# uthree/tinyvc

Measured on AMD Instinct MI355X. Metric: audio-samples/sec (16 kHz) end-to-end VC, higher is better.
Workload: dtype f32 (fp32 in / out / accumulate; channel contractions as two-term fp16 splits on v_mfma_f32_32x32x16_f16: 22-bit significands, three part-products per fp32 product)

## Files before the change

tinyvc_amd/csrc/decoder.hip:

```cpp
#include "conv3s.h"
#include "conv_s2.h"
#include "film_s2.h"
#include "gemm_s2.h"
#include "small_kernels.h"
#include "tvc_common.h"

namespace tvc {


__device__ __forceinline__ float div24k(float x) {
    const float r = 1.0f / 24000.0f;
    const float q0 = __fmul_rn(x, r);
    return fmaf(fmaf(-q0, 24000.0f, x), r, q0);
}

__device__ __forceinline__ double wave_incl_scan(double v, int lane) {
#pragma unroll
    for (int o = 1; o < 64; o <<= 1) {
        double u = __shfl_up(v, o);
        if (lane >= o) v += u;
    }
    return v;
}

static __global__ __launch_bounds__(256) void harm_frame_sum_kernel(const float* __restrict__ f0, double* __restrict__ csum,
                                                                    int T, float scale, RagDev rg) {
    const int b = blockIdx.y, lane = threadIdx.x & 63;
    const int t = 4 * blockIdx.x + (threadIdx.x >> 6);
    const int rs = T;
    long fbase = (long)b * T, cbase = (long)b * kHarm * T;
    if (rg.tb) {
        T = rg.tb[b];
        fbase = cbase = rg.pre[b];
        scale = __fdiv_rn((float)T, (float)(T * kHop));
    }
    if (t >= T) return;
    const float* f = f0 + fbase;
    double acc[kHarm];
#pragma unroll
    for (int m = 0; m < kHarm; ++m) acc[m] = 0.0;
    if (lane < kHop / 8) {
#pragma unroll
        for (int k = 0; k < 8; ++k) {
            Lerp c = lerp_coord(t * kHop + 8 * lane + k, scale, T);
            float fs = lerp_eval(c, f[c.i0], f[c.i1]);
#pragma unroll
            for (int m = 0; m < kHarm; ++m) acc[m] += (double)div24k(__fmul_rn(fs, (float)(m + 1)));
        }
    }
#pragma unroll
    for (int m = 0; m < kHarm; ++m) {
        double v = acc[m];
#pragma unroll
        for (int o = 32; o > 0; o >>= 1) v += __shfl_xor(v, o);
        if (lane == m) csum[cbase + (long)m * rs + t] = v;
    }
}

static __global__ __launch_bounds__(64) void harm_frame_scan_kernel(double* __restrict__ csum, int T, RagDev rg) {
    double* p = csum + ((long)blockIdx.y * kHarm + blockIdx.x) * T;
    if (rg.tb) {
        p = csum + (long)blockIdx.x * T + rg.pre[blockIdx.y];
        T = rg.tb[blockIdx.y];
    }
    const int lane = threadIdx.x;
    double carry = 0.0;
    for (int base = 0; base < T; base += 64) {
        int i = base + lane;
        double v = i < T ? p[i] : 0.0;
        double inc = wave_incl_scan(v, lane);
        if (i < T) p[i] = carry + (inc - v);
        carry += __shfl(inc, 63);
    }
}

static __global__ __launch_bounds__(256) void harm_synth_kernel(const float* __restrict__ f0, const float* __restrict__ amps,
                                                                const double* __restrict__ coff, float* __restrict__ source,
                                                                int T, float scale_size, float scale_amp, RagDev rg) {
    const int b = blockIdx.y, lane = threadIdx.x & 63;
    const int t = 4 * blockIdx.x + (threadIdx.x >> 6);
    const int rs = T;
    const long Ls = (long)T * kHop;
    long fbase = (long)b * T, abase = (long)b * kHarm * T, sbase = (long)b * 16 * Ls;
    if (rg.tb) {
        T = rg.tb[b];
        fbase = abase = rg.pre[b];
        sbase = (long)rg.pre[b] * kHop;
        scale_size = __fdiv_rn((float)T, (float)(T * kHop));
    }
    if (t >= T) return;
    const bool act = lane < kHop / 8;
    const float* f = f0 + fbase;
    const int p0 = t * kHop + 8 * (act ? lane : 0);
    float fs[8], uv[8];
    Lerp ca[8];
#pragma unroll
    for (int e = 0; e < 8; ++e) {
        const Lerp c = lerp_coord(p0 + e, scale_size, T);
        const float a0 = f[c.i0], a1 = f[c.i1];
        fs[e] = lerp_eval(c, a0, a1);
        uv[e] = lerp_eval(c, a0 > 20.f ? 1.f : 0.f, a1 > 20.f ? 1.f : 0.f);
        ca[e] = lerp_coord(p0 + e, scale_amp, T);
    }
    for (int m = 0; m < kHarm; ++m) {
        double d[8], sum = 0.0;
#pragma unroll
        for (int e = 0; e < 8; ++e) {
            d[e] = act ? (double)div24k(__fmul_rn(fs[e], (float)(m + 1))) : 0.0;
            sum += d[e];
        }
        const double inc = wave_incl_scan(sum, lane);
        double run = coff[abase + (long)m * rs + t] + (inc - sum);
        if (act) {
            const float* am = amps + abase + (long)m * rs;
            float o[8];
#pragma unroll
            for (int e = 0; e < 8; ++e) {
                run += d[e];
                const float I = (float)run;
                const float frac = I - floorf(I);
                const float theta = __fmul_rn(6.2831854820251465f, frac);
                const float hsin = __fmul_rn(sincos_small(theta).x, uv[e]);
                const float amp = lerp_eval(ca[e], am[ca[e].i0], am[ca[e].i1]);
                o[e] = __fmul_rn(hsin, amp);
            }
            float4* dst = reinterpret_cast<float4*>(source + sbase + (long)m * Ls + p0);
            dst[0] = make_float4(o[0], o[1], o[2], o[3]);
            dst[1] = make_float4(o[4], o[5], o[6], o[7]);
        }
    }
}

static __global__ __launch_bounds__(256) void noise_ola_kernel(const float* __restrict__ frames, float* __restrict__ source, int B, int T, float* __restrict__ smax, RagDev rg) {
    __shared__ float red[4];
    const long Ls = (long)T * kHop;
    const long b = blockIdx.y;
    long fbase = b * T, sbase = (b * 16 + 15) * Ls;
    if (rg.tb) {
        T = rg.tb[b];
        fbase = rg.pre[b];
        sbase = 15 * Ls + (long)rg.pre[b] * kHop;
    }
    const long L = (long)T * kHop;
    float mx = 0.f;
    for (long i = blockIdx.x * (long)blockDim.x + threadIdx.x; i < L; i += (long)gridDim.x * blockDim.x) {
        int p = (int)i;
        int q = p + kNfft / 2;
        int f_hi = q / kHop;
        if (f_hi > T) f_hi = T;
        int f_lo = (q - (kNfft - 1) + kHop - 1) / kHop;
        if (q - (kNfft - 1) <= 0) f_lo = 0;
        float s = 0.f;
        for (int f = f_lo > 1 ? f_lo : 1; f <= f_hi; ++f)
            s = __fadd_rn(s, frames[(fbase + (f - 1)) * kNfft + (q - f * kHop)]);
        const float v = s / (float)(f_hi - f_lo + 1);
        source[sbase + p] = v;
        mx = fmaxf(mx, fabsf(v));
    }
    amax_flush_wg(smax + b, mx, red);
}

static int run_source_net(tvc_ctx* ctx, hipStream_t s, Ws& ws, const float* content, const float* f0,
                          const float* energy, float* amps, float* kern, int B, int T, const float* cmax, float* xmax_zeroed, hipEvent_t amps_ready = nullptr) {
    const int ncols = B * T;
    float* ef = ws.get<float>((size_t)B * T);
    float* x = ws.get<float>((size_t)B * kSrcCh * T);
    const int NB = ctx->rag ? ctx->rag->B : B;
    float* xmax = xmax_zeroed ? xmax_zeroed : ws.get<float>((size_t)NB);
    if (!ws.dry) {
        hipLaunchKernelGGL(window_max_kernel, dim3(grid_for((long)ncols * 64)), dim3(256), 0, s, energy, ef, (long)B, T, kHop);
        EpiSumCond ep{x, ctx->src_content_in.bias, ef, f0, ctx->src_e_w, ctx->src_e_b, ctx->src_f_w, ctx->src_f_b, kSrcCh, T, ncols};
        int rc = 0;
        if (!gemm_s2_try(&rc, ctx, s, ctx->src_content_in, content, B, kSslDim, T, 0, ep, cmax)) rc = gemm_s_launch<2, 4, 2>(ctx, s, ctx->src_content_in, content, B, kSslDim, T, 0, ep, cmax);
        TVC_CHECK(rc);
    }
    if (!ws.dry && !xmax_zeroed) TVC_HIP(ctx, hipMemsetAsync(xmax, 0, (size_t)NB * sizeof(float), s));
    for (int i = 0; i < 3; ++i) TVC_CHECK(run_convnext(ctx, s, ws, ctx->src_mid[i], x, B, T, i == 2 ? xmax : nullptr));
    if (ws.dry) return 0;
    EpiBias<ACT_ELU1, false> ea{amps, ctx->src_to_amps.bias, nullptr, kHarm, T, ncols, (long)kHarm * T, 0};
    TVC_CHECK((gemm_s_launch<1, 4, 2>(ctx, s, ctx->src_to_amps, x, B, kSrcCh, T, 0, ea, xmax)));
    if (amps_ready) TVC_HIP(ctx, hipEventRecord(amps_ready, s));
    EpiBias<ACT_ELU1, false> ek{kern, ctx->src_to_kernel.bias, nullptr, kBins, T, ncols, (long)kBins * T, 0};
    TVC_CHECK((gemm_s_launch<2, 4, 2>(ctx, s, ctx->src_to_kernel, x, B, kSrcCh, T, 0, ek, xmax)));
    return launch_check(ctx, "source_net");
}

static int run_harm_sums(tvc_ctx* ctx, hipStream_t s, const float* f0, double* csum, int B, int T) {
    const long L = (long)T * kHop;
    const int NB = ctx->rag ? ctx->rag->B : B;
    const int Tg = ctx->rag ? ctx->rag->Tlong : T;
    RagDev rg;
    TVC_CHECK(rag_view(ctx, s, 1, 0, &rg, nullptr));
    const float scale_size = (float)T / (float)L;
    hipLaunchKernelGGL(harm_frame_sum_kernel, dim3((Tg + 3) / 4, NB), dim3(256), 0, s, f0, csum, T, scale_size, rg);
    hipLaunchKernelGGL(harm_frame_scan_kernel, dim3(kHarm, NB), dim3(64), 0, s, csum, T, rg);
    return launch_check(ctx, "harm_sums");
}

int run_dsp(tvc_ctx* ctx, hipStream_t s, Ws& ws, const float* f0, const float* amps, const float* kern, const float* angle, uint64_t seed, float* source, int B, int T,
            float* smax, double* csum, const DspFork* fk) {
    const long L = (long)T * kHop;
    if (!csum) csum = ws.get<double>((size_t)B * kHarm * T);
    float* frames = ws.get<float>((size_t)B * T * kNfft);
    const int NB = ctx->rag ? ctx->rag->B : B;
    const int Tg = ctx->rag ? ctx->rag->Tlong : T;
    float* smax_own = smax ? nullptr : ws.get<float>((size_t)NB);
    if (ws.dry) return 0;
    if (!smax) {
        smax = smax_own;
        TVC_HIP(ctx, hipMemsetAsync(smax, 0, (size_t)NB * sizeof(float), s));
    }
    RagDev rg;
    TVC_CHECK(rag_view(ctx, s, 1, 0, &rg, nullptr));
    const float scale_size = (float)T / (float)L;
    const float scale_amp = (float)(1.0 / (double)kHop);
    hipStream_t sh = s;
    if (fk) {
        sh = fk->side;
        TVC_HIP(ctx, hipStreamWaitEvent(sh, fk->amps_ready, 0));
    } else {
        TVC_CHECK(run_harm_sums(ctx, s, f0, csum, B, T));
    }
    hipLaunchKernelGGL(harm_synth_kernel, dim3((Tg + 3) / 4, NB), dim3(256), 0, sh, f0, amps, csum, source, T, scale_size, scale_amp, rg);
    TVC_CHECK(run_amax_rows(ctx, sh, amps, B, kHarm, T, smax));
    TVC_CHECK(run_noise_ifft(ctx, s, kern, angle, seed, frames, B, T, ctx->rag && angle));
    hipLaunchKernelGGL(noise_ola_kernel, dim3(grid_for((long)Tg * kHop / 4, 256, NB >= 32 ? 16 : 512 / NB), NB), dim3(256), 0, s, frames, source, B, T, smax, rg);
    return launch_check(ctx, "dsp");
}

static int plain_conv(tvc_ctx* ctx, hipStream_t s, const PackedW& w, const float* x, int B, int Cin, int len, int dil, float* y, const BfpSlots& bfp, int lin = 0,
                      float lscale = 0.f) {
    int rc = 0;
    if ((lin > 0 ? conv_s2_try<true>(&rc, ctx, s, w, x, B, Cin, len, dil, y, bfp, lin, lscale) : conv_s2_try<false>(&rc, ctx, s, w, x, B, Cin, len, dil, y, bfp)))
        return rc;
    if (lin > 0)
        return conv3s_launch<true, C3EpiBias<false>, false, true>(ctx, s, w, x, B, Cin, len, dil, C3EpiBias<false>{y, w.bias, nullptr, w.M, len}, bfp, nullptr, nullptr,
                                                                   nullptr, 0, lin, lscale);
    return conv3s_launch<true>(ctx, s, w, x, B, Cin, len, dil, C3EpiBias<false>{y, w.bias, nullptr, w.M, len}, bfp);
}

static int film_conv(tvc_ctx* ctx, hipStream_t s, const PackedW& w, const PackedW& fw, const FilmU& fu, const float* h, const float* cond, int B, int C, int len, int dil,
                     float* out, const float* bsc, const float* bsh, const float* res, int res_lin, float res_scale, const BfpSlots& bfp) {
    int rc = 0;
    if (rag_min_len(ctx, len) >= FS2::BN && film_s2_try(&rc, ctx, s, fu, h, cond, B, C, len, dil, out, res, res_lin, res_scale, bfp)) return rc;
    return conv3s_launch<true, C3EpiFilmFused, true>(ctx, s, w, h, B, C, len, dil, C3EpiFilmFused{out, w.bias, bsc, bsh, res, C, len, res_lin, res_scale}, bfp, &fw, &fw,
                                                     cond, C);
}

static int half_first(tvc_ctx* ctx, hipStream_t s, const PackedW& ca, const FilmU& fu, const float* x, int lin, float lscale, int da, int db, float* h, int B, int C, int len,
                      const float* res, int res_lin, const float* ma_in, float* mh, const float* mcond, bool* pre) {
    *pre = false;
    const bool can = rag_min_len(ctx, len) >= FS2::BN && fu.img && fu.C == C && fu.hb_w > 0.f && C % 96 == 0 && C <= 384 && ma_in && mcond && res && db >= 1 && db <= FS2::MAXD &&
                     (long)C * len * 4 < (1L << 32) && (res_lin <= 0 || (long)C * res_lin * 4 < (1L << 32));
    if (can) {
        int rc = 0;
        const BfpSlots in{ma_in, nullptr, nullptr};
        const bool ok = lin > 0 ? conv_s2_try<true, true>(&rc, ctx, s, ca, x, B, C, len, da, h, in, lin, lscale, fu.hb_w, fu.hb_b)
                                : conv_s2_try<false, true>(&rc, ctx, s, ca, x, B, C, len, da, h, in, 0, 0.f, fu.hb_w, fu.hb_b);
        if (ok) {
            *pre = rc == 0;
            return rc;
        }
    }
    return plain_conv(ctx, s, ca, x, B, C, len, da, h, BfpSlots{ma_in, nullptr, mh}, lin, lscale);
}

static int half_film(tvc_ctx* ctx, hipStream_t s, const PackedW& cb, const PackedW& fw, const FilmU& fu, int db, const float* h, const float* cond, int B, int C, int len,
                     float* out, const float* bsc, const float* bsh, const float* res, int res_lin, float res_scale, const float* ma_in, const float* mh, const float* mcond,
                     float* mout, bool pre) {
    if (pre) {
        int rc = 0;
        if (!film_s2_try(&rc, ctx, s, fu, h, cond, B, C, len, db, out, res, res_lin, res_scale, BfpSlots{ma_in, mcond, mout}, true, fu.hb_w, fu.hb_b))
            return fail(ctx, TVC_ERR_STATE, "filter_net: the FiLM conv refused the pre-split operand its producer wrote");
        return rc;
    }
    return film_conv(ctx, s, cb, fw, fu, h, cond, B, C, len, db, out, bsc, bsh, res, res_lin, res_scale, BfpSlots{mh, mcond, mout});
}

static int conv_film_half(tvc_ctx* ctx, hipStream_t s, const PackedW& ca, const PackedW& cb, const PackedW& fw, const FilmU& fu, const float* x, int lin, float lscale,
                          int da, int db, float* h, const float* cond, int B, int C, int len, float* out, const float* bsc, const float* bsh, const float* res,
                          int res_lin, float res_scale, const float* ma_in, float* mh, const float* mcond, float* mout) {
    bool pre = false;
    TVC_CHECK(half_first(ctx, s, ca, fu, x, lin, lscale, da, db, h, B, C, len, res, res_lin, ma_in, mh, mcond, &pre));
    return half_film(ctx, s, cb, fw, fu, db, h, cond, B, C, len, out, bsc, bsh, res, res_lin, res_scale, ma_in, mh, mcond, mout, pre);
}

constexpr int kHalfDil[2][2] = {{1, 3}, {9, 27}};

static __global__ void g8_to_planar_kernel(const float* __restrict__ x, float* __restrict__ y, long B, long l, int C) {
    const long n = B * C * l;
    for (long i = blockIdx.x * (long)blockDim.x + threadIdx.x; i < n; i += (long)gridDim.x * blockDim.x) {
        const long t = i % l, bc = i / l, c = bc % C, b = bc / C;
        y[i] = x[((b * (C / 8) + c / 8) * l + t) * 8 + (c & 7)];
    }
}

static int filter_input_gemm(tvc_ctx* ctx, hipStream_t s, const float* content, const float* f0, float* x, int B, int T, const float* cmax) {
    EpiSumCond ep{x, ctx->flt_content_in.bias, nullptr, f0, nullptr, nullptr, ctx->flt_f_w, ctx->flt_f_b, 384, T, B * T};
    int rc = 0;
    if (!gemm_s2_try(&rc, ctx, s, ctx->flt_content_in, content, B, kSslDim, T, 0, ep, cmax)) rc = gemm_s_launch<2, 4, 2>(ctx, s, ctx->flt_content_in, content, B, kSslDim, T, 0, ep, cmax);
    return rc;
}

int run_filter(tvc_ctx* ctx, hipStream_t s, Ws& ws, const float* content, const float* f0,
               const float* energy, const float* source, float* wave, int B, int T, const FilterTaps* taps, const float* cmax, const float* smax, float* zeroed_slots, bool x_slot_set,
               const FilterFront* front) {
    const long L = (long)T * kHop;
    static const int ch[5] = {384, 192, 96, 48, 24};
    const long len_dn[5] = {L, L / 5, L / 20, L / 80, L / 240};
    float* skip[5];
    for (int i = 0; i < 5; ++i) skip[i] = ws.get<float>((size_t)B * ch[4 - i] * len_dn[i]);
    float* x = front ? front->x0 : ws.get<float>((size_t)B * ch[0] * T);
    const UpW& u0 = ctx->ups[0];
    const int lo0 = T * u0.factor;
    float* h0 = front ? front->h0 : ws.get<float>((size_t)B * u0.cin * lo0);
    SideFork* fk = front && front->fk && front->fk->forked() ? front->fk : nullptr;
    bool pre0 = false;
    float* xi_pre[5] = {nullptr, nullptr, nullptr, nullptr, nullptr};
    for (int i = 1; i <= 4; ++i) xi_pre[i] = ws.get<float>((size_t)B * ctx->downs[i - 1].cin * len_dn[i]);
    for (int i = 1; i < 4; ++i)
        if (len_dn[i] % ctx->downs[i].factor != 0 || (ctx->downs[i].factor == 4 && len_dn[i] % 4 != 0))
            return fail(ctx, TVC_ERR_ARG, "filter_net: level lengths must divide by the next Downsample factor");

    enum { S_CONTENT = 0, S_SRC, S_X, S_SKIP0, S_DH1 = S_SKIP0 + 5, S_DH2 = S_DH1 + 4, S_UHA = S_DH2 + 4, S_UX1 = S_UHA + 5, S_UHB = S_UX1 + 5, S_UXU = S_UHB + 5,
           S_LEV = S_UXU + 5, S_COUNT = S_LEV + 5 };
    const int NB = ctx->rag ? ctx->rag->B : B;
    static_assert(S_COUNT == kFilterSlots && S_X == kFilterSlotX, "tvc_common.h kFilterSlots / kFilterSlotX");
    float* slots = zeroed_slots ? zeroed_slots : ws.get<float>((size_t)S_COUNT * NB);
    auto slot = [&](int i) { return slots + (size_t)i * NB; };
    auto up0_first = [&](hipStream_t st) {
        return half_first(ctx, st, u0.c1, u0.fu1, x, T, (float)(1.0 / (double)u0.factor), kHalfDil[0][0], kHalfDil[0][1], h0, B, u0.cin, lo0, x, T, slot(S_X), slot(S_UHA),
                          slot(S_SKIP0 + 4), &pre0);
    };

    if (!ws.dry) {
        ProfScope ps(ctx, s, ws, "filter.in+down0");
        if (!zeroed_slots) TVC_HIP(ctx, hipMemsetAsync(slots, 0, (size_t)S_COUNT * NB * sizeof(float), s));
        if (!cmax) {
            TVC_CHECK(run_amax_rows(ctx, s, content, B, kSslDim, T, slot(S_CONTENT)));
            cmax = slot(S_CONTENT);
        }
        if (!smax) {
            TVC_CHECK(run_amax_rows(ctx, s, source, B, 16, L, slot(S_SRC)));
            TVC_CHECK(run_amax_rows(ctx, s, energy, B, 1, L, slot(S_SRC)));
            smax = slot(S_SRC);
        }
        if (fk && !(zeroed_slots && x_slot_set)) return fail(ctx, TVC_ERR_STATE, "filter_net: a forked front needs its slots prepared in front of the fork");
        if (!fk) TVC_CHECK(filter_input_gemm(ctx, s, content, f0, x, B, T, cmax));
        if (!(zeroed_slots && x_slot_set)) TVC_CHECK(run_slot_affine(ctx, s, slot(S_X), cmax, 1, ctx->flt_in_bw, ctx->flt_in_bb, NB));
        if (fk) {
            {
                ProfScope ps(ctx, fk->side, ws, "filter_net.input@side");
                TVC_CHECK(up0_first(fk->side));
            }
            TVC_CHECK(fk->end());
        }
        TVC_CHECK(run_down0_split(ctx, s, ctx->flt_down0s, source, energy, skip[0], taps ? taps->skips[0] : nullptr, xi_pre[1], B, (int)L, smax, slot(S_SKIP0)));
    }
    for (int i = 1; i <= 4; ++i) {
        const DownW& d = ctx->downs[i - 1];
        const int len = (int)len_dn[i];
        size_t mk = ws.mark();
        float* xi = xi_pre[i];
        float* h1 = d.cin == 24 ? nullptr : ws.get<float>((size_t)B * d.cin * len);
        float* h2 = d.cin == 24 ? nullptr : ws.get<float>((size_t)B * d.cin * len);
        if (!ws.dry) {
            static const char* names[4] = {"filter.down1", "filter.down2", "filter.down3", "filter.down4"};
            ProfScope ps(ctx, s, ws, names[i - 1]);
            float* y2 = i < 4 ? xi_pre[i + 1] : nullptr;
            const int f2 = i < 4 ? ctx->downs[i].factor : 0;
            const float* mxi = slot(S_SKIP0 + i - 1);
            float *mh1 = slot(S_DH1 + i - 1), *mh2 = slot(S_DH2 + i - 1), *mout = slot(S_SKIP0 + i);
            if (d.cin == 24) {
                TVC_CHECK(run_down24_fused(ctx, s, d, xi, skip[i], y2, B, len, mxi, mout));
            } else {
                if (d.cin == 48) {
                    TVC_CHECK(run_conv48_pair(ctx, s, d.c1, d.c2, xi, 0, 0.f, nullptr, nullptr, nullptr, nullptr, h2, B, len, 1, 2, mxi, nullptr, mh2));
                } else {
                    TVC_CHECK(plain_conv(ctx, s, d.c1, xi, B, d.cin, len, 1, h1, BfpSlots{mxi, nullptr, mh1}));
                    TVC_CHECK(plain_conv(ctx, s, d.c2, h1, B, d.cin, len, 2, h2, BfpSlots{mh1, nullptr, mh2}));
                }
                TVC_CHECK((conv3s_launch<true, C3EpiBiasResConv>(ctx, s, d.c3, h2, B, d.cin, len, 4,
                                                                 C3EpiBiasResConv{{skip[i], d.c3res_bias, nullptr, d.cout, len, y2, f2}},
                                                                 BfpSlots{mh2, mxi, mout}, &d.res, nullptr, xi, d.cin)));
            }
        }
        ws.release(mk);
    }
    float* xlev[5];
    {
        long l = T;
        for (int i = 0; i < 5; ++i) {
            l *= ctx->ups[i].factor;
            xlev[i] = ws.get<float>((size_t)B * ctx->ups[i].cout * l);
        }
    }
    long len = T;
    const float* mx_in = slot(S_X);
    for (int i = 0; i < 5; ++i) {
        const UpW& u = ctx->ups[i];
        const int lin = (int)len;
        len *= u.factor;
        const int lo = (int)len, C = u.cin, nc = B * lo;
        const float* cond = skip[4 - i];
        const float* mcond = slot(S_SKIP0 + 4 - i);
        size_t mk = ws.mark();
        float* xu = ws.get<float>((size_t)B * C * lo);
        float* h = i == 0 ? h0 : ws.get<float>((size_t)B * C * lo);
        float* x1 = ws.get<float>((size_t)B * C * lo);
        if (!ws.dry && C == 24) {
            ProfScope ps(ctx, s, ws, "filter.up4+out");
            TVC_CHECK(run_up24_split(ctx, s, u, x, cond, ctx->down0_bw, ctx->down0_bb, x1, wave, B, lo, mx_in, smax, slot(S_UX1 + i)));
        } else if (!ws.dry) {
            static const char* names[4] = {"filter.up0", "filter.up1", "filter.up2", "filter.up3"};
            ProfScope ps(ctx, s, ws, names[i]);
            const float lscale = (float)(1.0 / (double)u.factor);
            for (int half = 0; half < 2; ++half) {
                const PackedW& ca = half ? u.c3 : u.c1;
                const PackedW& cb = half ? u.c4 : u.c2;
                const PackedW& fw = half ? u.film2 : u.film1;
                const float* bsc = fw.bias;
                const float* bsh = fw.bias + C;
                const int da = kHalfDil[half][0], db = kHalfDil[half][1];
                float* xout = half ? xu : x1;
                const float* ma_in = half ? slot(S_UX1 + i) : mx_in;
                float* mh = slot((half ? S_UHB : S_UHA) + i);
                float* mout = slot((half ? S_UXU : S_UX1) + i);
                if (C == 48) {
                    if (half == 0) {
                        TVC_CHECK(run_conv48_pair(ctx, s, ca, cb, x, lin, lscale, &fw, bsc, bsh, cond, xout, B, lo, da, db, ma_in, mcond, mout));
                    } else {
                        TVC_CHECK(run_conv48s(ctx, s, ca, x1, nullptr, nullptr, nullptr, nullptr, nullptr, h, B, lo, da, ma_in, nullptr, mh));
                        TVC_CHECK(run_conv48s(ctx, s, cb, h, &fw, bsc, bsh, cond, x1, nullptr, B, lo, db, mh, mcond, slot(S_LEV + i), &u.c5, xlev[i]));
                    }
                } else if (half == 0 && i == 0) {
                    if (fk) TVC_CHECK(fk->join());
                    else TVC_CHECK(up0_first(s));
                    TVC_CHECK(half_film(ctx, s, cb, fw, u.fu1, db, h, cond, B, C, lo, xout, bsc, bsh, x, lin, lscale, ma_in, mh, mcond, mout, pre0));
                } else if (half == 0) {
                    TVC_CHECK(conv_film_half(ctx, s, ca, cb, fw, u.fu1, x, lin, lscale, da, db, h, cond, B, C, lo, xout, bsc, bsh, x, lin, lscale, ma_in, mh, mcond, mout));
                } else {
                    TVC_CHECK(conv_film_half(ctx, s, ca, cb, fw, u.fu2, x1, 0, 0.f, da, db, h, cond, B, C, lo, xout, bsc, bsh, x1, 0, 0.f, ma_in, mh, mcond, mout));
                }
            }
            if (C != 48) {
                EpiBias<ACT_NONE, false> ep{xlev[i], u.c5.bias, nullptr, u.cout, lo, nc, (long)u.cout * lo, 0, slot(S_LEV + i), slot(S_UXU + i), u.c5_bw, u.c5_bb, NB};
                if (u.cout == 48) {
                    EpiBiasG8 eg{xlev[i], u.c5.bias, u.cout, lo, nc, slot(S_LEV + i), slot(S_UXU + i), u.c5_bw, u.c5_bb, NB};
                    TVC_CHECK((gemm_s_launch<2, 4, 2>(ctx, s, u.c5, xu, B, C, lo, 0, eg, slot(S_UXU + i))));
                } else if (u.c5.MT6 % 3 == 0) TVC_CHECK((gemm_s_launch<3, 4, 1>(ctx, s, u.c5, xu, B, C, lo, 0, ep, slot(S_UXU + i))));
                else TVC_CHECK((gemm_s_launch<2, 4, 2>(ctx, s, u.c5, xu, B, C, lo, 0, ep, slot(S_UXU + i))));
            }
        }
        ws.release(mk);
        x = xlev[i];
        mx_in = slot(S_LEV + i);
    }
    if (!ws.dry && taps) {
        for (int i = 1; i < 5; ++i)
            if (taps->skips[i] && i == 1)
                hipLaunchKernelGGL(g8_to_planar_kernel, dim3(grid_for((long)B * 48 * len_dn[1])), dim3(256), 0, s, skip[1], taps->skips[1], (long)B, len_dn[1], 48);
            else if (taps->skips[i])
                TVC_HIP(ctx, hipMemcpyAsync(taps->skips[i], skip[i], (size_t)B * ch[4 - i] * len_dn[i] * sizeof(float), hipMemcpyDeviceToDevice, s));
        long l = T;
        for (int i = 0; i < 4; ++i) {
            l *= ctx->ups[i].factor;
            if (taps->ups[i] && ctx->ups[i].cout <= 48)
                hipLaunchKernelGGL(g8_to_planar_kernel, dim3(grid_for((long)B * ctx->ups[i].cout * l)), dim3(256), 0, s, xlev[i], taps->ups[i], (long)B, l, ctx->ups[i].cout);
            else if (taps->ups[i])
                TVC_HIP(ctx, hipMemcpyAsync(taps->ups[i], xlev[i], (size_t)B * ctx->ups[i].cout * l * sizeof(float), hipMemcpyDeviceToDevice, s));
        }
    }
    return ws.dry ? 0 : launch_check(ctx, "filter_net");
}

int run_decoder(tvc_ctx* ctx, hipStream_t s, Ws& ws, const float* content, const float* f0,
                const float* energy, const float* angle, uint64_t seed, float* wave, float* amps_out,
                float* kernel_out, float* source_out, int B, int T, const float* content_bound, const float* energy_bound,
                int content_bound_stride) {
    const long L = (long)T * kHop;
    float* amps = amps_out ? amps_out : ws.get<float>((size_t)B * kHarm * T);
    float* kern = kernel_out ? kernel_out : ws.get<float>((size_t)B * kBins * T);
    float* source = source_out ? source_out : ws.get<float>((size_t)B * 16 * L);
    const int NB = ctx->rag ? ctx->rag->B : B;
    float* cmax = ws.get<float>((size_t)(3 + kFilterSlots) * NB);
    float* smax = cmax + NB;
    float* xmax = smax + NB;
    float* fslots = xmax + NB;
    float* x0 = ws.get<float>((size_t)B * 384 * T);
    float* h0 = ws.get<float>((size_t)B * ctx->ups[0].cin * T * ctx->ups[0].factor);
    double* csum = ws.get<double>((size_t)B * kHarm * T);
    if (!ws.dry) {
        TVC_CHECK(run_slot_prep(ctx, s, cmax, (3 + kFilterSlots) * NB, content_bound ? cmax : nullptr, content_bound, content_bound_stride, 1.f, 0.f, energy_bound ? smax : nullptr,
                                energy_bound, 1, 1.f, 0.f, content_bound ? fslots + (size_t)kFilterSlotX * NB : nullptr, ctx->flt_in_bw, ctx->flt_in_bb,
                                NB));
        if (!content_bound) TVC_CHECK(run_amax_rows(ctx, s, content, B, kSslDim, T, cmax));
        if (!energy_bound) TVC_CHECK(run_amax_rows(ctx, s, energy, B, 1, L, smax));
        if (!content_bound && wave) TVC_CHECK(run_slot_affine(ctx, s, fslots + (size_t)kFilterSlotX * NB, cmax, 1, ctx->flt_in_bw, ctx->flt_in_bb, NB));
        if (wave && ctx->rag) {
            RagDev rd;
            TVC_CHECK(rag_tiles(ctx, s, B, (long)T * ctx->ups[0].factor, CS2::BN, &rd, nullptr, "filter_net front"));
        }
    }
    SideFork fk(ctx, s);
    if (wave) TVC_CHECK(fk.fork(ws, ctx->ev_fork2, ctx->ev_join2));
    const FilterFront front{&fk, x0, h0};
    if (fk.forked()) {
        TVC_CHECK(run_harm_sums(ctx, fk.side, f0, csum, B, T));
        ProfScope ps(ctx, fk.side, ws, "filter_net.input@side");
        TVC_CHECK(filter_input_gemm(ctx, fk.side, content, f0, x0, B, T, cmax));
    }
    size_t mk = ws.mark();
    {
        ProfScope ps(ctx, s, ws, "source_net");
        TVC_CHECK(run_source_net(ctx, s, ws, content, f0, energy, amps, kern, B, T, cmax, xmax, fk.forked() ? ctx->ev_amps : nullptr));
    }
    ws.release(mk);
    if (!wave && !source_out) return 0;
    {
        ProfScope ps(ctx, s, ws, "dsp");
        const DspFork df{fk.side, ctx->ev_amps};
        TVC_CHECK(run_dsp(ctx, s, ws, f0, amps, kern, angle, seed, source, B, T, smax, csum, fk.forked() ? &df : nullptr));
        TVC_CHECK(fk.join_so_far(ctx->ev_src));
    }
    ws.release(mk);
    if (!wave) return 0;
    ProfScope ps(ctx, s, ws, "filter_net");
    TVC_CHECK(run_filter(ctx, s, ws, content, f0, energy, source, wave, B, T, nullptr, cmax, smax, fslots, true, &front));
    ws.release(mk);
    return 0;
}

}
```

tinyvc_amd/csrc/encoder.hip:

```cpp
#include "conv3s.h"
#include "gemm_s2.h"
#include "cnx_s3.h"
#include "small_kernels.h"
#include "tvc_common.h"

namespace tvc {

constexpr int ENC_MTB = 4, ENC_NWV = 4, ENC_BPC = 2;

template <bool DW, int CPT>
static __global__ __launch_bounds__(1024) void dwconv_ln_kernel(const float* x, float* y,
                                                               const float* __restrict__ dw_w, const float* __restrict__ dw_b,
                                                               const float* __restrict__ g, const float* __restrict__ bta,
                                                               int C, int T, int dil, RagDev rg) {
    constexpr int NW = 16;
    const int rs = T;
    long ubase = (long)blockIdx.y * C * T;
    if (rg.tb) {
        T = rg.tb[blockIdx.y];
        ubase = rg.pre[blockIdx.y];
        if ((int)blockIdx.x * 64 >= T) return;
    }
    __shared__ float red[NW][64];
    constexpr bool STAGE = CPT >= 16;
    __shared__ __attribute__((aligned(16))) float Wl[STAGE ? 16 * CPT * 8 : 8];
    __shared__ float Gl[2][STAGE ? 16 * CPT : 1];
    if (STAGE) {
        for (int i = threadIdx.x; i < C; i += 1024) {
            if (DW) {
#pragma unroll
                for (int j = 0; j < 7; ++j) Wl[i * 8 + j] = dw_w[i * 7 + j];
                Wl[i * 8 + 7] = dw_b[i];
            }
            Gl[0][i] = g[i];
            Gl[1][i] = bta[i];
        }
        __syncthreads();
    }
    const int lane = threadIdx.x & 63, wave = threadIdx.x >> 6;
    const int t = blockIdx.x * 64 + lane;
    const bool ok = t < T;
    const int tc = ok ? t : T - 1;
    const float* xb = x + ubase;
    float* yb = y + ubase;

    int tt[7];
#pragma unroll
    for (int j = 0; j < 7; ++j) {
        int q = tc + (j - 3) * dil;
        tt[j] = q < 0 ? 0 : (q >= T ? T - 1 : q);
    }
    float v[CPT];
    float sum = 0.f;
#pragma unroll
    for (int i = 0; i < CPT; ++i) {
        const int c = wave + i * NW;
        if (DW) {
            const float* xr = xb + (long)c * rs;
            float wj[7], a;
            if (STAGE) {
                const float4 w0 = *reinterpret_cast<const float4*>(Wl + c * 8), w1 = *reinterpret_cast<const float4*>(Wl + c * 8 + 4);
                wj[0] = w0.x; wj[1] = w0.y; wj[2] = w0.z; wj[3] = w0.w; wj[4] = w1.x; wj[5] = w1.y; wj[6] = w1.z;
                a = w1.w;
            } else {
#pragma unroll
                for (int j = 0; j < 7; ++j) wj[j] = dw_w[c * 7 + j];
                a = dw_b[c];
            }
#pragma unroll
            for (int j = 0; j < 7; ++j) a = fmaf(wj[j], xr[tt[j]], a);
            v[i] = a;
        } else {
            v[i] = xb[(long)c * rs + tc];
        }
        sum += v[i];
    }
    red[wave][lane] = sum;
    __syncthreads();
    float tot = 0.f;
#pragma unroll
    for (int w = 0; w < NW; ++w) tot += red[w][lane];
    const float mean = tot / (float)C;
    __syncthreads();
    float sq = 0.f;
#pragma unroll
    for (int i = 0; i < CPT; ++i) {
        const float d = v[i] - mean;
        sq = fmaf(d, d, sq);
    }
    red[wave][lane] = sq;
    __syncthreads();
    float tot2 = 0.f;
#pragma unroll
    for (int w = 0; w < NW; ++w) tot2 += red[w][lane];
    const float var = tot2 / (float)C;
    const float rstd = 1.f / sqrtf(var + 1e-5f);
    if (!ok) return;
#pragma unroll
    for (int i = 0; i < CPT; ++i) {
        const int c = wave + i * NW;
        yb[(long)c * rs + t] = fmaf((v[i] - mean) * rstd, STAGE ? Gl[0][c] : g[c], STAGE ? Gl[1][c] : bta[c]);
    }
}
template <bool DW>
static int dwconv_ln_launch(tvc_ctx* ctx, hipStream_t s, const float* x, float* y, const float* dw_w, const float* dw_b, const float* g,
                            const float* bta, int B, int C, int T, int dil) {
    RagDev rg;
    TVC_CHECK(rag_view(ctx, s, 1, 0, &rg, nullptr));
    const dim3 grid(((ctx->rag ? ctx->rag->Tlong : T) + 63) / 64, ctx->rag ? ctx->rag->B : B), blk(1024);
    if (C == 384) hipLaunchKernelGGL((dwconv_ln_kernel<DW, 24>), grid, blk, 0, s, x, y, dw_w, dw_b, g, bta, C, T, dil, rg);
    else if (C == 128) hipLaunchKernelGGL((dwconv_ln_kernel<DW, 8>), grid, blk, 0, s, x, y, dw_w, dw_b, g, bta, C, T, dil, rg);
    else return fail(ctx, TVC_ERR_ARG, "dwconv_ln: unsupported channel count %d", C);
    return 0;
}

static __global__ void grn_norm_kernel(const float* __restrict__ h, float* __restrict__ gx, long rows, int T, RagDev rg, int C2) {
    const int lane = threadIdx.x & 63;
    long wave = (blockIdx.x * (long)blockDim.x + threadIdx.x) >> 6;
    long nwaves = ((long)gridDim.x * blockDim.x) >> 6;
    for (long r = wave; r < rows; r += nwaves) {
        const float* p = h + r * T;
        int n = T;
        if (rg.tb) {
            const int b = (int)(r / C2), c = (int)(r - (long)b * C2);
            p = h + (long)c * T + rg.pre[b];
            n = rg.tb[b];
        }
        float s = 0.f;
        for (int t = lane; t < n; t += 64) s = fmaf(p[t], p[t], s);
#pragma unroll
        for (int o = 32; o > 0; o >>= 1) s += __shfl_xor(s, o);
        if (lane == 0) gx[r] = sqrtf(s);
    }
}

static __global__ __launch_bounds__(256) void grn_finalize_kernel(const float* __restrict__ gx, const float* __restrict__ gamma,
                                                                  float* __restrict__ nx, int C2, float* __restrict__ hmax) {
    __shared__ float red[4];
    __shared__ float redm[4];
    const int b = blockIdx.x;
    const float* g = gx + (long)b * C2;
    float s = 0.f;
    for (int c = threadIdx.x; c < C2; c += 256) s += g[c];
#pragma unroll
    for (int o = 32; o > 0; o >>= 1) s += __shfl_xor(s, o);
    if ((threadIdx.x & 63) == 0) red[threadIdx.x >> 6] = s;
    __syncthreads();
    const float mean = (red[0] + red[1] + red[2] + red[3]) / (float)C2;
    const float den = mean + 1e-6f;
    float mx = 0.f;
    for (int c = threadIdx.x; c < C2; c += 256) {
        const float f = fmaf(gamma[c], g[c] / den, 1.f);
        nx[(long)b * C2 + c] = f;
        mx = fmaxf(mx, g[c] * fabsf(f));
    }
#pragma unroll
    for (int o = 32; o > 0; o >>= 1) mx = fmaxf(mx, __shfl_xor(mx, o));
    if ((threadIdx.x & 63) == 0) redm[threadIdx.x >> 6] = mx;
    __syncthreads();
    if (threadIdx.x == 0) hmax[b] = fmaxf(fmaxf(redm[0], redm[1]), fmaxf(redm[2], redm[3]));
}

int run_layernorm(tvc_ctx* ctx, hipStream_t s, float* x, const float* g, const float* b, int B, int C, int T) {
    TVC_CHECK(dwconv_ln_launch<false>(ctx, s, x, x, nullptr, nullptr, g, b, B, C, T, 1));
    return launch_check(ctx, "layernorm");
}

static __global__ void grn_tiles_kernel(float* __restrict__ gp, int gp_tiles, int K, int T, RagDev rg) {
    const int b = blockIdx.y, c = blockIdx.x * blockDim.x + threadIdx.x;
    if (c >= K) return;
    const int Tb = rg.tb ? rg.tb[b] : T, n = (Tb + 63) / 64;
    float* g = gp + (long)b * gp_tiles * K + c;
    float s = g[0];
    for (int t = 1; t < n; ++t) s += g[(long)t * K];
    g[0] = s;
}

template <int C>
static bool cnx_try(int* rc, tvc_ctx* ctx, hipStream_t s, const ConvNeXtW& w, float* x, float* h, float* gx, int B, int T, float* amax_out) {
    if (w.C != C || !(w.ln_bound < 32768.f) || w.c2.MT6 != 2 * C / 32 || w.c3.MT6 != C / 32 || w.c2.S6 < C / 16 || w.c3.S6 < 2 * C / 16) return false;
    const int NB = ctx->rag ? ctx->rag->B : B, Tl = ctx->rag ? ctx->rag->Tlong : T, rs = T;
    if ((long)rs * 8 * 4 >= (1L << 31)) return false;
    constexpr int KP = C == 384 ? 2 : 1;
    if ((*rc = lds_optin<cnx1_kernel<C, 1>>(ctx, Cnx1<C, 1>::LDS_BYTES, "cnx")) ||
        (*rc = lds_optin<cnx1_kernel<C, 2>>(ctx, Cnx1<C, 2>::LDS_BYTES, "cnx")) ||
        (*rc = lds_optin<cnx2_kernel<C, KP>>(ctx, Cnx2<C, KP>::LDS_BYTES, "cnx")))
        return true;
    CnxArgs a{};
    a.x = x;
    a.h = h;
    a.T = T;
    a.rs = rs;
    if ((*rc = rag_view(ctx, s, 1, 0, &a.rg, nullptr)) != 0) return true;
    auto split = [&](int MT, int tiles) {
        int d = 1;
        for (int c = 1; c <= MT; ++c)
            if (MT % c == 0 && (long)tiles * c <= ctx->ncu) d = c;
        return d;
    };
    {
        a.A6 = reinterpret_cast<const uint4*>(w.c2.A6);
        a.wsc = w.c2.wscale;
        a.bias = w.c2.bias;
        a.MT = w.c2.MT6;
        a.dw_w = w.dw_w;
        a.dw_b = w.dw_b;
        a.ln_g = w.ln_g;
        a.ln_b = w.ln_b;
        a.dil = w.dilation;
        const int nt = Tl <= 32 ? 1 : 2, tx = (Tl + 32 * nt - 1) / (32 * nt);
        a.gp = gx;
        a.gp_tiles = tx;
        const int d = split(a.MT, tx * NB);
        a.mt_per_wg = a.MT / d;
        const dim3 grid((unsigned)tx, (unsigned)NB, (unsigned)d);
        constexpr int nthr = Cnx1<C, 2>::NTHR, lds1 = Cnx1<C, 1>::LDS_BYTES, lds2 = Cnx1<C, 2>::LDS_BYTES;
        if (nt == 1) hipLaunchKernelGGL((cnx1_kernel<C, 1>), grid, dim3(nthr), lds1, s, a);
        else hipLaunchKernelGGL((cnx1_kernel<C, 2>), grid, dim3(nthr), lds2, s, a);
    }
    a.gp_sum = a.gp_tiles > CNX_GP_INLINE;
    if (a.gp_sum) hipLaunchKernelGGL(grn_tiles_kernel, dim3((2 * C + 255) / 256, (unsigned)NB), dim3(256), 0, s, gx, a.gp_tiles, 2 * C, T, a.rg);
    {
        a.A6 = reinterpret_cast<const uint4*>(w.c3.A6);
        a.wsc = w.c3.wscale;
        a.bias = w.c3_bias_grn;
        a.MT = w.c3.MT6;
        a.grn_g = w.grn_g;
        a.amax_y = amax_out;
        const int tx = (Tl + 63) / 64;
        const int d = split(a.MT, tx * NB);
        a.mt_per_wg = a.MT / d;
        constexpr int nthr = Cnx2<C, KP>::NTHR, lds = Cnx2<C, KP>::LDS_BYTES;
        hipLaunchKernelGGL((cnx2_kernel<C, KP>), dim3((unsigned)tx, (unsigned)NB, (unsigned)d), dim3(nthr), lds, s, a);
    }
    *rc = launch_check(ctx, "convnext (fused)");
    return true;
}

int run_convnext(tvc_ctx* ctx, hipStream_t s, Ws& ws, const ConvNeXtW& w, float* x, int B, int T, float* amax_out) {
    const int C = w.C, C2 = 2 * w.C, ncols = B * T;
    const int NB = ctx->rag ? ctx->rag->B : B;
    size_t mk = ws.mark();
    float* y = ws.get<float>((size_t)B * C * T);
    float* h = ws.get<float>((size_t)B * C2 * T);
    const int Tlong = ctx->rag ? ctx->rag->Tlong : T;
    float* gx = ws.get<float>((size_t)NB * C2 * ((Tlong + 63) / 64));
    float* nx = ws.get<float>((size_t)NB * C2);
    float* ymax = ws.get<float>((size_t)NB);
    float* hmax = ws.get<float>((size_t)NB);
    ws.release(mk);
    if (ws.dry) return 0;
    {
        int rc = 0;
        if (C == 384 ? cnx_try<384>(&rc, ctx, s, w, x, h, gx, B, T, amax_out) : (C == 128 && cnx_try<128>(&rc, ctx, s, w, x, h, gx, B, T, amax_out))) return rc;
    }
    {
        TVC_CHECK(dwconv_ln_launch<true>(ctx, s, x, y, w.dw_w, w.dw_b, w.ln_g, w.ln_b, B, C, T, w.dilation));
    }
    {
        const float* ym = nullptr;
        if (!(w.ln_bound < 32768.f)) {
            TVC_HIP(ctx, hipMemsetAsync(ymax, 0, (size_t)NB * sizeof(float), s));
            TVC_CHECK(run_amax_rows(ctx, s, y, B, C, T, ymax));
            ym = ymax;
        }
        EpiBias<ACT_GELU, false> ep{h, w.c2.bias, nullptr, C2, T, ncols, (long)C2 * T, 0};
        int rc = 0;
        if (!gemm_s2_try(&rc, ctx, s, w.c2, y, B, C, T, 0, ep, ym)) rc = gemm_s_launch<ENC_MTB, ENC_NWV, ENC_BPC>(ctx, s, w.c2, y, B, C, T, 0, ep, ym);
        TVC_CHECK(rc);
    }
    {
        RagDev rg;
        TVC_CHECK(rag_view(ctx, s, 1, 0, &rg, nullptr));
        hipLaunchKernelGGL(grn_norm_kernel, dim3(grid_for((long)NB * C2 * 64)), dim3(256), 0, s, h, gx, (long)NB * C2, T, rg, C2);
        hipLaunchKernelGGL(grn_finalize_kernel, dim3(NB), dim3(256), 0, s, gx, w.grn_g, nx, C2, hmax);
    }
    {
        EpiBias<ACT_NONE, true> ep{x, w.c3_bias_grn, x, C, T, ncols, (long)C * T, (long)C * T};
        int rc = 0;
        if (!gemm_s2_try<EpiBias<ACT_NONE, true>, true>(&rc, ctx, s, w.c3, h, B, C2, T, 0, ep, hmax, nx))
            rc = gemm_s_launch<ENC_MTB, ENC_NWV, ENC_BPC, EpiBias<ACT_NONE, true>, true>(ctx, s, w.c3, h, B, C2, T, 0, ep, hmax, nx);
        TVC_CHECK(rc);
    }
    if (amax_out) TVC_CHECK(run_amax_rows(ctx, s, x, B, C, T, amax_out));
    return launch_check(ctx, "convnext");
}

struct EpiSplit {
    static constexpr bool kIgemm = true;
    float* y0;
    float* y1;
    const float* bias;
    int M0, M1, T, ncols;
    __device__ __forceinline__ void store(int n, int m, const float v[4]) const {
        if (n >= ncols) return;
        int b = n / T, t = n - b * T;
#pragma unroll
        for (int r = 0; r < 4; ++r) {
            int mm = m + r;
            float o = v[r] + bias[mm < M0 + M1 ? mm : 0];
            if (mm < M0)
                y0[((long)b * M0 + mm) * T + t] = o;
            else if (mm < M0 + M1)
                y1[((long)b * M1 + mm - M0) * T + t] = o;
        }
    }
};

struct PTop4 {
    float v[4];
    int i[4];
    __device__ __forceinline__ void init() {
#pragma unroll
        for (int j = 0; j < 4; ++j) { v[j] = -INFINITY; i[j] = 0x7fffffff; }
    }
    __device__ __forceinline__ static bool better(float a, int ia, float b, int ib) { return a > b || (a == b && ia < ib); }
    __device__ __forceinline__ void insert(float x, int ix) {
        if (!better(x, ix, v[3], i[3])) return;
        if (better(x, ix, v[0], i[0])) { v[3] = v[2]; i[3] = i[2]; v[2] = v[1]; i[2] = i[1]; v[1] = v[0]; i[1] = i[0]; v[0] = x; i[0] = ix; }
        else if (better(x, ix, v[1], i[1])) { v[3] = v[2]; i[3] = i[2]; v[2] = v[1]; i[2] = i[1]; v[1] = x; i[1] = ix; }
        else if (better(x, ix, v[2], i[2])) { v[3] = v[2]; i[3] = i[2]; v[2] = x; i[2] = ix; }
        else { v[3] = x; i[3] = ix; }
    }
};

constexpr int kPdWaves = 16;
static __global__ __launch_bounds__(kPdWaves * 64) void pitch_decode_kernel(const float* __restrict__ logits, const float* __restrict__ freq,
                                                                  float* __restrict__ f0, int B, int T, float* __restrict__ f0s, float shift,
                                                                  const float* __restrict__ shifts, const int* __restrict__ col2b) {
    __shared__ float sv[kPdWaves][4][64];
    __shared__ int si[kPdWaves][4][64];
    const int lane = threadIdx.x & 63, wave = threadIdx.x >> 6;
    const long ncols = (long)B * T;
    const long n = blockIdx.x * 64L + lane;
    const bool ok = n < ncols;
    const long nn = ok ? n : ncols - 1;
    const int b = (int)(nn / T), t = (int)(nn - (long)b * T);
    const float* p = logits + (long)b * kPitchClasses * T + t;
    PTop4 top;
    top.init();
    constexpr int CPW = kPitchClasses / kPdWaves;
    float xv[CPW];
#pragma unroll
    for (int j = 0; j < CPW; ++j) xv[j] = p[(long)(wave * CPW + j) * T];
#pragma unroll
    for (int j = 0; j < CPW; ++j) {
        const float x = xv[j];
        top.insert(x != x ? INFINITY : x, wave * CPW + j);
    }
#pragma unroll
    for (int e = 0; e < 4; ++e) { sv[wave][e][lane] = top.v[e]; si[wave][e][lane] = top.i[e]; }
    __syncthreads();
    if (wave != 0 || !ok) return;
    for (int w = 1; w < kPdWaves; ++w)
#pragma unroll
        for (int e = 0; e < 4; ++e) top.insert(sv[w][e][lane], si[w][e][lane]);
#pragma unroll
    for (int e = 0; e < 4; ++e) top.i[e] = (unsigned)top.i[e] < (unsigned)kPitchClasses ? top.i[e] : 0;
    const float v0 = top.v[0];
    float e0 = 1.f, e1 = (float)exp((double)(top.v[1] - v0)), e2 = (float)exp((double)(top.v[2] - v0)), e3 = (float)exp((double)(top.v[3] - v0));
    float den = ((e0 + e1) + e2) + e3;
    float acc = __fmul_rn(e0 / den, freq[top.i[0]]);
    acc = __fadd_rn(acc, __fmul_rn(e1 / den, freq[top.i[1]]));
    acc = __fadd_rn(acc, __fmul_rn(e2 / den, freq[top.i[2]]));
    acc = __fadd_rn(acc, __fmul_rn(e3 / den, freq[top.i[3]]));
    const float fv = acc <= 20.f ? 0.f : acc;
    f0[n] = fv;
    if (f0s) f0s[n] = shift_frequency_one(fv, shifts ? shifts[col2b ? col2b[n] : b] : shift);
}

int run_pitch_decode(tvc_ctx* ctx, hipStream_t s, const float* logits, float* f0, int B, int T) {
    if (!ctx->pitch_freq) return fail(ctx, TVC_ERR_STATE, "pitch table not uploaded (tvc_set_pitch_table + tvc_finalize_weights)");
    const long ncols = (long)B * T;
    hipLaunchKernelGGL(pitch_decode_kernel, dim3((unsigned)((ncols + 63) / 64)), dim3(kPdWaves * 64), 0, s, logits, ctx->pitch_freq, f0, B, T, (float*)nullptr, 0.f, (const float*)nullptr, (const int*)nullptr);
    return launch_check(ctx, "pitch_decode");
}

int run_encoder(tvc_ctx* ctx, hipStream_t s, Ws& ws, const float* spec, float* ssl, float* f0,
                float* logits, int B, int T, const float* spec_bound, float* zeroed_slots, float* f0_shifted, float shift, const float* shifts) {
    const int ncols = B * T;
    float* xs = ws.get<float>((size_t)B * kSslCh * T);
    float* xp = ws.get<float>((size_t)B * kPitchCh * T);
    float* lg = logits ? logits : ws.get<float>((size_t)B * kPitchClasses * T);
    const int NB = ctx->rag ? ctx->rag->B : B;
    float* slots = zeroed_slots ? zeroed_slots : ws.get<float>((size_t)3 * NB);
    float *spec_max = slots, *xs_max = slots + NB, *xp_max = slots + 2 * NB;
    if (!ws.dry) {
        if (!zeroed_slots) TVC_HIP(ctx, hipMemsetAsync(slots, 0, (size_t)3 * NB * sizeof(float), s));
        if (spec_bound) spec_max = const_cast<float*>(spec_bound);
        else TVC_CHECK(run_amax_rows(ctx, s, spec, B, kBins, T, spec_max));
        EpiSplit ep{xs, xp, ctx->enc_in.bias, kSslCh, kPitchCh, T, ncols};
        TVC_CHECK((gemm_s_launch_ragged<ENC_MTB, ENC_NWV, ENC_BPC>(ctx, s, ctx->enc_in, spec, B, kBins, T, (long)kBins * T, ep, spec_max)));
        TVC_CHECK(run_layernorm(ctx, s, xs, ctx->ssl_ln_g, ctx->ssl_ln_b, B, kSslCh, T));
        TVC_CHECK(run_layernorm(ctx, s, xp, ctx->pit_ln_g, ctx->pit_ln_b, B, kPitchCh, T));
    }
    const int gtiles = ((ctx->rag ? ctx->rag->Tlong : T) + 63) / 64;
    const size_t ssl_scratch = ((size_t)B * kSslCh * T * 3 + (size_t)NB * kSslCh * 2 * (gtiles + 1)) * sizeof(float) + (size_t)NB * 8 + 4096;
    char* ssl_blk = ws.get<char>(ssl_scratch);
    Ws wssl(ssl_blk, ssl_scratch, ws.dry);
    SideFork fk(ctx, s);
    TVC_CHECK(fk.fork(ws, ctx->ev_fork, ctx->ev_join));
    const hipStream_t sp = fk.side;
    for (int i = 0; i < 4; ++i) TVC_CHECK(run_convnext(ctx, sp, ws, ctx->pit_mid[i], xp, B, T, i == 3 ? xp_max : nullptr));
    if (!ws.dry) {
        EpiBias<ACT_NONE, false> ep{lg, ctx->pit_out.bias, nullptr, kPitchClasses, T, ncols, (long)kPitchClasses * T, 0};
        int rc = 0;
        if (!gemm_s2_try(&rc, ctx, sp, ctx->pit_out, xp, B, kPitchCh, T, 0, ep, xp_max)) rc = gemm_s_launch<ENC_MTB, ENC_NWV, ENC_BPC>(ctx, sp, ctx->pit_out, xp, B, kPitchCh, T, 0, ep, xp_max);
        TVC_CHECK(rc);
        hipLaunchKernelGGL(pitch_decode_kernel, dim3((ncols + 63) / 64), dim3(kPdWaves * 64), 0, sp, lg, ctx->pitch_freq, f0, B, T, f0_shifted, shift, shifts,
                           shifts && ctx->rag ? ctx->rag->d_col2b : (const int*)nullptr);
    }
    TVC_CHECK(fk.end());
    for (int i = 0; i < 6; ++i) TVC_CHECK(run_convnext(ctx, s, wssl, ctx->ssl_mid[i], xs, B, T, i == 5 ? xs_max : nullptr));
    if (wssl.peak > wssl.cap) return fail(ctx, TVC_ERR_WORKSPACE, "encoder: SSL scratch block too small");
    if (ws.dry) return 0;
    {
        EpiBias<ACT_NONE, false> ep{ssl, ctx->ssl_out.bias, nullptr, kSslDim, T, ncols, (long)kSslDim * T, 0};
        int rc = 0;
        if (!gemm_s2_try(&rc, ctx, s, ctx->ssl_out, xs, B, kSslCh, T, 0, ep, xs_max)) rc = gemm_s_launch<ENC_MTB, ENC_NWV, ENC_BPC>(ctx, s, ctx->ssl_out, xs, B, kSslCh, T, 0, ep, xs_max);
        TVC_CHECK(rc);
    }
    TVC_CHECK(fk.join());
    return launch_check(ctx, "encoder");
}

int run_ssl_amax(tvc_ctx* ctx, hipStream_t s, const float* ssl, int B, int T, float* slot) { return run_amax_rows(ctx, s, ssl, B, kSslDim, T, slot); }

}
```

Measured before the change: 726.4 million.

## Add output-stationary GEMM that keeps the whole split input tile in LDS

After: 726.3 million. About the same (-0.0%).

```diff
diff --git a/tinyvc_amd/csrc/decoder.hip b/tinyvc_amd/csrc/decoder.hip
--- a/tinyvc_amd/csrc/decoder.hip
+++ b/tinyvc_amd/csrc/decoder.hip
@@ -1,6 +1,7 @@
 #include "conv3s.h"
 #include "conv_s2.h"
 #include "film_s2.h"
+#include "gemm_os.h"
 #include "gemm_s2.h"
 #include "small_kernels.h"
 #include "tvc_common.h"
@@ -181,7 +182,9 @@
     TVC_CHECK((gemm_s_launch<1, 4, 2>(ctx, s, ctx->src_to_amps, x, B, kSrcCh, T, 0, ea, xmax)));
     if (amps_ready) TVC_HIP(ctx, hipEventRecord(amps_ready, s));
     EpiBias<ACT_ELU1, false> ek{kern, ctx->src_to_kernel.bias, nullptr, kBins, T, ncols, (long)kBins * T, 0};
-    TVC_CHECK((gemm_s_launch<2, 4, 2>(ctx, s, ctx->src_to_kernel, x, B, kSrcCh, T, 0, ek, xmax)));
+    int rc = 0;
+    if (!gemm_os_try<kSrcCh, 8>(&rc, ctx, s, ctx->src_to_kernel, x, B, kSrcCh, T, ek, xmax)) rc = gemm_s_launch<2, 4, 2>(ctx, s, ctx->src_to_kernel, x, B, kSrcCh, T, 0, ek, xmax);
+    TVC_CHECK(rc);
     return launch_check(ctx, "source_net");
 }
 
@@ -448,8 +451,12 @@
                 if (u.cout == 48) {
                     EpiBiasG8 eg{xlev[i], u.c5.bias, u.cout, lo, nc, slot(S_LEV + i), slot(S_UXU + i), u.c5_bw, u.c5_bb, NB};
                     TVC_CHECK((gemm_s_launch<2, 4, 2>(ctx, s, u.c5, xu, B, C, lo, 0, eg, slot(S_UXU + i))));
-                } else if (u.c5.MT6 % 3 == 0) TVC_CHECK((gemm_s_launch<3, 4, 1>(ctx, s, u.c5, xu, B, C, lo, 0, ep, slot(S_UXU + i))));
-                else TVC_CHECK((gemm_s_launch<2, 4, 2>(ctx, s, u.c5, xu, B, C, lo, 0, ep, slot(S_UXU + i))));
+                } else {
+                    int rc = 0;
+                    if (gemm_os_try<384, 6>(&rc, ctx, s, u.c5, xu, B, C, lo, ep, slot(S_UXU + i)) || gemm_os_try<192, 3>(&rc, ctx, s, u.c5, xu, B, C, lo, ep, slot(S_UXU + i))) TVC_CHECK(rc);
+                    else if (u.c5.MT6 % 3 == 0) TVC_CHECK((gemm_s_launch<3, 4, 1>(ctx, s, u.c5, xu, B, C, lo, 0, ep, slot(S_UXU + i))));
+                    else TVC_CHECK((gemm_s_launch<2, 4, 2>(ctx, s, u.c5, xu, B, C, lo, 0, ep, slot(S_UXU + i))));
+                }
             }
         }
         ws.release(mk);
diff --git a/tinyvc_amd/csrc/encoder.hip b/tinyvc_amd/csrc/encoder.hip
--- a/tinyvc_amd/csrc/encoder.hip
+++ b/tinyvc_amd/csrc/encoder.hip
@@ -1,6 +1,7 @@
 #include "conv3s.h"
 #include "gemm_s2.h"
 #include "cnx_s3.h"
+#include "gemm_os.h"
 #include "small_kernels.h"
 #include "tvc_common.h"
 
@@ -417,7 +418,8 @@
     {
         EpiBias<ACT_NONE, false> ep{ssl, ctx->ssl_out.bias, nullptr, kSslDim, T, ncols, (long)kSslDim * T, 0};
         int rc = 0;
-        if (!gemm_s2_try(&rc, ctx, s, ctx->ssl_out, xs, B, kSslCh, T, 0, ep, xs_max)) rc = gemm_s_launch<ENC_MTB, ENC_NWV, ENC_BPC>(ctx, s, ctx->ssl_out, xs, B, kSslCh, T, 0, ep, xs_max);
+        if (!gemm_os_try<kSslCh, 8>(&rc, ctx, s, ctx->ssl_out, xs, B, kSslCh, T, ep, xs_max) && !gemm_s2_try(&rc, ctx, s, ctx->ssl_out, xs, B, kSslCh, T, 0, ep, xs_max))
+            rc = gemm_s_launch<ENC_MTB, ENC_NWV, ENC_BPC>(ctx, s, ctx->ssl_out, xs, B, kSslCh, T, 0, ep, xs_max);
         TVC_CHECK(rc);
     }
     TVC_CHECK(fk.join());
diff --git a/tinyvc_amd/csrc/gemm_os.h b/tinyvc_amd/csrc/gemm_os.h
--- /dev/null
+++ b/tinyvc_amd/csrc/gemm_os.h
@@ -0,0 +1,165 @@
+#pragma once
+#include "cnx_s3.h"
+
+namespace tvc {
+
+struct GemmOsArgs {
+    const float* x;
+    int T, rs;
+    RagDev rg;
+    const uint4* A6;
+    const float* wsc;
+    const float* amax_x;
+    int MT, mt_per_wg;
+};
+
+template <int K, int WAVES_>
+struct GemmOs {
+    static constexpr int NT = 2, NC = 64, KS = K / 16, WAVES = WAVES_, NTHR = WAVES * 64;
+    static constexpr int GROUPS = K / 8, XPER = GROUPS / WAVES;
+    static constexpr int YS_U4 = KS * 4 * NC, MT_MAX = 32;
+    static constexpr int LDS_BYTES = YS_U4 * 16 + MT_MAX * 32 * 4;
+    static constexpr int QUADS = NT * 4;
+    static_assert(GROUPS % WAVES == 0, "staging items divide");
+    static_assert(KS >= QUADS, "an item's epilogue leaves within the next item's walk");
+    static_assert(LDS_BYTES <= 160 * 1024, "LDS");
+};
+
+template <int K, int WAVES, class Epi>
+__global__ __launch_bounds__((GemmOs<K, WAVES>::NTHR)) void gemm_os_kernel(GemmOsArgs a, Epi ep) {
+    using CF = GemmOs<K, WAVES>;
+    constexpr int NT = CF::NT, NC = CF::NC, KS = CF::KS, XPER = CF::XPER, QUADS = CF::QUADS;
+    extern __shared__ __attribute__((aligned(16))) uint4 smem_os[];
+    uint4* Ys = smem_os;
+    const int tid = threadIdx.x, lane = tid & 63, l31 = lane & 31, lh = lane >> 5;
+    const int wave = __builtin_amdgcn_readfirstlane(tid >> 6);
+    const int b = blockIdx.y;
+    int Tb = a.T, noff = b * a.T;
+    long xoff = (long)b * K * a.T;
+    if (a.rg.tb) {
+        Tb = a.rg.tb[b] * a.rg.mult;
+        noff = a.rg.pre[b] * a.rg.mult;
+        xoff = noff;
+    }
+    const int ntu = (Tb + NC - 1) / NC;
+    if ((int)blockIdx.x >= ntu) return;
+    const int TW = (Tb + ntu - 1) / ntu;
+    const int t0 = blockIdx.x * TW;
+    const int tw = Tb - t0 < TW ? Tb - t0 : TW;
+    const int rs = a.rs;
+    const Bfp sx = bfp_load(a.amax_x, b);
+    const int mt_lo = blockIdx.z * a.mt_per_wg;
+    const int mt_hi = mt_lo + a.mt_per_wg < a.MT ? mt_lo + a.mt_per_wg : a.MT;
+    float* Bl = reinterpret_cast<float*>(smem_os + CF::YS_U4);
+    for (int i = tid; i < (mt_hi - mt_lo) * 32; i += CF::NTHR) Bl[i] = ep.bias[mt_lo * 32 + i];
+    ep.bias = Bl - mt_lo * 32;
+
+    {
+        const float* xb = a.x + xoff;
+        const unsigned so = 4u * (unsigned)(t0 + (lane < tw ? lane : tw - 1));
+        float xr[XPER][8];
+#pragma unroll
+        for (int i = 0; i < XPER; ++i) {
+            const int gg = wave + i * WAVES;
+#pragma unroll
+            for (int q = 0; q < 8; ++q) xr[i][q] = ldg_so(xb + (long)(8 * gg + q) * rs, so);
+        }
+#pragma unroll
+        for (int i = 0; i < XPER; ++i) {
+            const int gg = wave + i * WAVES;
+#pragma unroll
+            for (int q = 0; q < 8; ++q) xr[i][q] *= sx.s;
+            uint4 p1, p2;
+            split8(xr[i], p1, p2);
+            Ys[(((gg >> 1) * 2 + 0) * 2 + (gg & 1)) * NC + lane] = p1;
+            Ys[(((gg >> 1) * 2 + 1) * 2 + (gg & 1)) * NC + lane] = p2;
+        }
+    }
+    __syncthreads();
+
+    int mt = mt_lo + wave;
+    if (mt >= mt_hi) return;
+    u32x4 ring[CNX_PD][2];
+#pragma unroll
+    for (int u = 0; u < CNX_PD; ++u) {
+        const uint4* ab = a.A6 + ((long)u * a.MT + mt) * kPU4;
+        ring[u][0] = ldg_so4(ab, 16u * (unsigned)lane);
+        ring[u][1] = ldg_so4(ab, 16u * (unsigned)(64 + lane));
+    }
+    int nn[NT];
+#pragma unroll
+    for (int j = 0; j < NT; ++j) {
+        const int n = j * 32 + l31;
+        nn[j] = noff + t0 + (n < tw ? n : tw - 1);
+    }
+    float pend[NT * 16];
+    int pmt = mt;
+    auto finish4 = [&](int e) __attribute__((always_inline)) {
+        const int j = e >> 2, q = e & 3;
+        float v[4] = {pend[16 * j + 4 * q], pend[16 * j + 4 * q + 1], pend[16 * j + 4 * q + 2], pend[16 * j + 4 * q + 3]};
+        asm volatile("" : "+v"(v[0]), "+v"(v[1]), "+v"(v[2]), "+v"(v[3]));
+        ep.store(nn[j], pmt * 32 + 8 * q + 4 * lh, v);
+    };
+    auto post = [&](int k) __attribute__((always_inline)) {
+        if (k < QUADS) finish4(k);
+    };
+    auto walk = [&](auto& poster) __attribute__((always_inline)) {
+        const int mtn = mt + WAVES < mt_hi ? mt + WAVES : mt;
+        f32x16 hi[NT], lo[NT];
+#pragma unroll
+        for (int j = 0; j < NT; ++j)
+#pragma unroll
+            for (int r = 0; r < 16; ++r) hi[j][r] = lo[j][r] = 0.f;
+        cnx_mma<NT, NC, KS>(hi, lo, ring, a.A6, a.MT, mt, 0, mtn, 0, Ys, lane, poster);
+        const float cw = sload_f32(a.wsc + mt) * sx.inv, cl = cw * kLoInv;
+#pragma unroll
+        for (int j = 0; j < NT; ++j)
+#pragma unroll
+            for (int r = 0; r < 16; ++r) pend[j * 16 + r] = comb(hi[j][r], lo[j][r], cw, cl);
+        pmt = mt;
+    };
+    {
+        CnxNoPost none;
+        walk(none);
+    }
+    while (mt + WAVES < mt_hi) {
+        mt += WAVES;
+        walk(post);
+    }
+#pragma unroll
+    for (int e = 0; e < QUADS; ++e) finish4(e);
+}
+
+template <int K, int WAVES, class Epi>
+inline int gemm_os_launch_t(tvc_ctx* ctx, hipStream_t s, const PackedW& w, const float* x, int B, int T, const Epi& ep, const float* amax_x) {
+    using CF = GemmOs<K, WAVES>;
+    TVC_CHECK((lds_optin<gemm_os_kernel<K, WAVES, Epi>>(ctx, CF::LDS_BYTES, "gemm_os")));
+    GemmOsArgs a{};
+    a.x = x;
+    a.T = T;
+    a.rs = T;
+    TVC_CHECK(rag_tiles(ctx, s, B, T, 0, &a.rg, nullptr, "gemm_os"));
+    a.A6 = reinterpret_cast<const uint4*>(w.A6);
+    a.wsc = w.wscale;
+    a.amax_x = amax_x;
+    a.MT = w.MT6;
+    const int NB = ctx->rag ? ctx->rag->B : B, Tl = ctx->rag ? ctx->rag->Tlong * a.rg.mult : T;
+    const int tx = (Tl + CF::NC - 1) / CF::NC;
+    int d = (int)(ctx->ncu / ((long)tx * NB));
+    const int dmax = (a.MT + WAVES - 1) / WAVES;
+    d = d < 1 ? 1 : (d > dmax ? dmax : d);
+    a.mt_per_wg = ((a.MT + d - 1) / d + WAVES - 1) / WAVES * WAVES;
+    d = (a.MT + a.mt_per_wg - 1) / a.mt_per_wg;
+    hipLaunchKernelGGL((gemm_os_kernel<K, WAVES, Epi>), dim3((unsigned)tx, (unsigned)NB, (unsigned)d), dim3(CF::NTHR), CF::LDS_BYTES, s, a, ep);
+    return launch_check(ctx, "gemm_os");
+}
+
+template <int K, int WAVES, class Epi>
+inline bool gemm_os_try(int* rc, tvc_ctx* ctx, hipStream_t s, const PackedW& w, const float* x, int B, int Cin, int T, const Epi& ep, const float* amax_x) {
+    static_assert(K == 128 || K == 192 || K == 384, "the whole split operand tile stays in LDS");
+    if (Cin != K || K / 16 > w.S6 || w.MT6 < 1 || w.MT6 > GemmOs<K, WAVES>::MT_MAX || (WAVES < 8 && w.MT6 > WAVES) || B < 1 || T < 1 || (long)B * T >= (1L << 29)) return false;
+    *rc = gemm_os_launch_t<K, WAVES, Epi>(ctx, s, w, x, B, T, ep, amax_x);
+    return true;
+}
+
+}
```
